# Guilucand/PanDelos

Hardware: AMD Instinct MI355X
Metric: scored gene-pairs/sec (whole node) (higher is better)
Workload: dtype u32 accumulate + f32 finalize

## Files before the change

### pandelos_amd/csrc/pdl_api.hip

```cpp
#include "pdl_common.h"

#include <algorithm>
#include <cstdlib>
#include <cstring>
#include <limits>

static thread_local std::string g_create_error = "";


static void check_genes(const char *who, const uint8_t *residues, const uint64_t *offsets, uint32_t n) {
    if (!offsets) PDL_FAIL(PDL_ERR_ARGUMENT, "%s: NULL pointer", who);
    if (n == 0) PDL_FAIL(PDL_ERR_ARGUMENT, "%s: no gene", who);
    for (uint32_t i = 0; i < n; i++)
        if (offsets[i + 1] < offsets[i]) PDL_FAIL(PDL_ERR_ARGUMENT, "%s: offsets decrease at gene %u", who, i);
    if (!residues && offsets[n] > offsets[0]) PDL_FAIL(PDL_ERR_ARGUMENT, "%s: NULL residues", who);
}

static void check_batch(const pdl_ctx *c, const char *who, const void *out, const uint8_t *residues, const uint64_t *offsets, const uint32_t *gene_begin,
                        uint32_t n, uint32_t n_queries) {
    if (n_queries == 0) PDL_FAIL(PDL_ERR_ARGUMENT, "%s: no query", who);
    if (n == 0) PDL_FAIL(PDL_ERR_ARGUMENT, "%s: no query gene", who);
    if (!out || !offsets || !gene_begin) PDL_FAIL(PDL_ERR_ARGUMENT, "%s: NULL pointer", who);
    if (gene_begin[0] != 0) PDL_FAIL(PDL_ERR_ARGUMENT, "%s: gene_begin[0] = %u, not 0", who, gene_begin[0]);
    for (uint32_t q = 0; q < n_queries; q++)
// ... 744 lines not shown
}

int pdl_set_option(pdl_ctx *c, const char *name, int64_t value) {
    if (!c || !name) return PDL_ERR_ARGUMENT;
    std::lock_guard<std::mutex> lk(c->mu);
    return guarded(c, [&]() -> int {
    const std::string n(name);
    if (n == "join_tier1") {
        if (!(value == -1 || value == 0 || (value >= 9 && value <= 11) || value == 20 || value == 21)) PDL_FAIL(PDL_ERR_ARGUMENT, "join_tier1: -1, 0, 9, 10, 11, 20 or 21");
        c->opt_tier1 = (int) value;
    } else if (n == "join_tier0") c->opt_tier0 = value < 0 ? -1 : (value != 0);
    else if (n == "sift_threshold") {
        if (value != 0 && value != 1) PDL_FAIL(PDL_ERR_ARGUMENT, "sift_threshold: 0 or 1");
        c->opt_sift_threshold = (int) value;
    }
    else if (n == "join_tiny_tier2") c->opt_tiny_tier2 = value != 0;
    else if (n == "join_grid_pct") c->opt_grid_pct = (int) value;
    else if (n == "stage_timers") c->opt_stage_timers = value != 0;
    else if (n == "host_mirror") c->opt_host_mirror = value != 0;
    else if (n == "staging_cap") c->opt_staging_cap = value > 0 ? (uint64_t) value : 0;
    else if (n == "aside_test_reload") c->opt_aside_test_reload = value != 0;
    else if (n == "onepass_scan") c->opt_onepass_scan = value != 0;
    else if (n == "lean_radix") c->opt_lean_radix = value != 0;
    else if (n == "low_memory") c->opt_low_memory = value != 0;
    else if (n == "query_batch_bytes") {
        if (value <= 0) PDL_FAIL(PDL_ERR_ARGUMENT, "query_batch_bytes: a positive byte count");
        c->opt_query_batch_bytes = (uint64_t) value;
        return PDL_OK;
    }
    else if (n == "query_rekey") {
        if (value != 0 && value != 1) PDL_FAIL(PDL_ERR_ARGUMENT, "query_rekey: 0 or 1");
        c->opt_query_rekey = value != 0;
        return PDL_OK;
    }
    else if (n == "alphabet_rekey") {
        if (value != 0 && value != 1) PDL_FAIL(PDL_ERR_ARGUMENT, "alphabet_rekey: 0 or 1");
        c->opt_alphabet_rekey = value != 0;
        return PDL_OK;
    }
    else throw pdl_error{PDL_ERR_ARGUMENT, "unknown option " + n};
    pdl_stale(c, Stale::scores);
    return PDL_OK;
    });
}

int pdl_dist_preprocess_begin(pdl_ctx *c, const uint8_t *d_residues, const uint64_t *d_offsets, const uint32_t *d_genome_of,
// ... 274 lines not shown
```

### pandelos_amd/csrc/pdl_common.h

```cpp
#pragma once

#include <atomic>
#include <chrono>

#include <hip/hip_runtime.h>

#include <algorithm>
#include <cstdint>
#include <cstdio>
#include <mutex>
#include <cstdlib>
#include <new>
#include <string>
#include <utility>
#include <vector>

#include "../../include/pandelos_amd.h"

#define PDL_WAVE 64

#ifdef __HIPCC__
__device__ __forceinline__ void pdl_sync() {
#ifndef PDL_PLAIN_SYNCTHREADS
    asm volatile("s_waitcnt lgkmcnt(0)" ::: "memory");
#endif
    __syncthreads();
}
#endif

enum : size_t {
    PDL_CTL_RECORDS = 0,
    PDL_CTL_FREE_1 = 1,
    PDL_CTL_RANGES = 2,
    PDL_CTL_BAD_OFFSETS = 3,
    PDL_CTL_KSEQ_SUM = 4,
    PDL_CTL_KMERS = 5,
    PDL_CTL_EMITTED = 6,
    PDL_CTL_KSEQ_MAX = 7,
    PDL_CTL_KSEQ_NMIN = 8,
    PDL_CTL_MIRRORED = 9,
    PDL_CTL_COUNTERS = 10,
    PDL_CTL_SHARED = 10,
// ... 276 lines not shown

    DevBuf kseq_len;
    DevBuf gene_len;
    DevBuf kmer_off;
    DevBuf cost;
    std::vector<uint64_t> h_genome_cost;

    DevBuf keys_a, keys_b, vals_a, vals_b, sort_tmp;
    bool key64 = false;
    DevBuf recpos;
    DevBuf post;
    DevBuf ranges;
    const uint2 *ranges8 = nullptr;
    DevBuf head_bits;
    bool costs_ready = true;
    DevBuf seq_off;
    bool upper_only = false;
    DevBuf scan_tmp;
    DevBuf lb_tile, lb_chunk, lb_ctr;
    uint32_t lb_epoch = 0;
    bool opt_low_memory = false;
    bool reshard_pending = false;
    bool opt_onepass_scan = false;
    bool opt_lean_radix = true;
    DevBuf scratch;
    DevBuf scalars;

    std::vector<uint32_t> h_genome_of;
    std::vector<uint32_t> h_genome_row_off;
    std::vector<uint32_t> h_genome_rows;
    std::vector<uint32_t> shard;
    bool shard_set = false;
    std::vector<uint32_t> dict_shard;
    DevBuf seq_in_shard;
    DevBuf own_iv;
    std::vector<uint2> h_own_iv;
    std::vector<uint8_t> h_seq_in_shard;

    bool scored = false;
    uint32_t n_task_rows = 0;
    std::vector<int32_t> h_local_genome;
    std::vector<uint32_t> h_task_row_off;
    std::vector<uint64_t> h_cell_off;
    DevBuf task_blob;
    uint32_t *task_pin = nullptr; size_t task_pin_words = 0;
    hipStream_t copy_stream = nullptr; hipEvent_t ev_tasks = nullptr, ev_entry = nullptr;
// ... 391 lines not shown
```

### pandelos_amd/csrc/pdl_dict.hip

```cpp
#include "pdl_common.h"
#include "pdl_scan.h"
#include "pdl_sort.h"
#include "pdl_append.h"
#include "pdl_remove.h"
#include "pdl_rekey.h"
#include "pdl_groups.h"

#include <algorithm>
#include <cstring>


__global__ __launch_bounds__(256) void k_zero_u64(uint64_t *p, size_t n) {
    for (size_t i = (size_t) blockIdx.x * 256 + threadIdx.x; i < n; i += (size_t) gridDim.x * 256) p[i] = 0;
}
constexpr int HIST_THREADS = 256;
__global__ __launch_bounds__(HIST_THREADS) void k_hist(const uint8_t *__restrict__ res, uint64_t n, unsigned long long *__restrict__ hist) {
    __shared__ uint32_t s_seen[256];
    s_seen[threadIdx.x] = 0;
    pdl_sync();
    const uint64_t n16 = n / 16;
    const uint4 *res16 = reinterpret_cast<const uint4 *>(res);
    const uint64_t stride = (uint64_t) gridDim.x * HIST_THREADS;
    auto mark = [&](const uint4 &v) {
        const uint32_t w[4] = {v.x, v.y, v.z, v.w};
// ... 649 lines not shown
    c->tm.sort_seq_ms = ev_ms(c, EV_SORT2); c->tm.ranges_ms = ev_ms(c, EV_RANGES);
    return ev_ms(c, total_event);
}

static void stage_ranges_and_costs(pdl_ctx *c, uint64_t bound, int mode, bool only_complexity) {
    uint64_t *d_scal = c->scalars.as<uint64_t>();
    GroupPlan gp = group_tiles_plan(c, pdl_postings(c), bound, d_scal + PDL_CTL_RECORDS);
    gp.a.cost = c->cost.as<unsigned long long>();
    gp.a.counters = reinterpret_cast<unsigned long long *>(d_scal + PDL_CTL_COUNTERS);
    hipLaunchKernelGGL(k_fold_last_record, dim3(1), dim3(1024), 0, c->stream, gp.a.post, c->post_ext ? (uint32_t *) nullptr : c->recpos.as<uint32_t>(), gp.a.d_n);
    if (only_complexity) { c->ranges8 = nullptr; launch_group_costs<false, true>(c, gp.a, gp.grid); }
    else build_ranges(c, gp.a, gp.grid, mode);
    c->costs_ready = c->ranges8 == nullptr;
    launch_genome_cost(c, PDL_CTL_KSEQ_SUM, PDL_CTL_KSEQ_MAX);
    PinRead rd(c);
    const uint64_t *pt = closing_read(c, rd, PDL_CTL_GCOST + (size_t) c->G);
    c->h_genome_cost.assign(pt + PDL_CTL_GCOST, pt + PDL_CTL_GCOST + c->G);
    c->U = pt[PDL_CTL_RECORDS]; c->Ushared = pt[PDL_CTL_SHARED]; c->Urepeat = pt[PDL_CTL_REPEATS]; c->NG = pt[PDL_CTL_GROUPS];
    c->P = c->costs_ready ? 0 : pt[PDL_CTL_OWN_COST];
    if (c->costs_ready) for (uint64_t v : c->h_genome_cost) c->P += v;
}

void pdl_run_reshard(pdl_ctx *c) {
    hipStream_t st = c->stream;
    if (c->dist || c->post_ext) PDL_FAIL(PDL_ERR_STATE, "genome shard: a multi-GPU context deals the genomes itself");
    if (c->dict_shard.empty() || c->upper_only) PDL_FAIL(PDL_ERR_STATE, "genome shard: the dictionary was built for all genomes; set the first shard before pdl_preprocess");
    const uint32_t n = (uint32_t) c->U;
    ev_begin(c, EV_PRE_TOTAL);
    hipLaunchKernelGGL(k_restore_heads, dim3((n + 255) / 256), dim3(256), 0, st, c->post.as<uint2>(), c->head_bits.as<unsigned long long>(), n);
    clear_ctl(c, PDL_CTL_RANGES, PDL_CTL_RANGES);
    clear_ctl(c, PDL_CTL_COUNTERS, PDL_CTL_LAST);
    clear_genome_words(c);
    clear_gene_costs(c);
    const uint64_t sum_kseq = c->sum_kseq, max_kseq = c->max_kseq, min_kseq = c->min_kseq;
    clear_kseq_stats(c);
    c->dict_shard = c->shard;
    c->tasks_ready = false;
    ev_begin(c, EV_DICT); ev_end(c, EV_DICT);
    stage_ranges_and_costs(c, c->U, 0, false);
    c->sum_kseq = sum_kseq; c->max_kseq = max_kseq; c->min_kseq = min_kseq;
    ev_end(c, EV_PRE_TOTAL);
    c->tm.reshard_ms = close_range_timings(c, EV_PRE_TOTAL);
}

void pdl_ensure_costs(pdl_ctx *c) {
    if (c->costs_ready) return;
    hipStream_t st = c->stream;
    uint64_t *d_scal = c->scalars.as<uint64_t>();
    clear_gene_costs(c);
    clear_genome_words(c, false);
    const uint32_t n = (uint32_t) c->U;
    hipLaunchKernelGGL(k_gene_costs_lazy, dim3((n + 255) / 256), dim3(256), 0, st, pdl_postings(c), c->head_bits.as<unsigned long long>(), n,
// ... 688 lines not shown
```

### pandelos_amd/csrc/pdl_groups.h

```cpp
#pragma once
#include "pdl_common.h"
#include "pdl_scan.h"
#include "pdl_sort.h"

constexpr uint32_t HEAD_BIT = 0x80000000u;
constexpr uint32_t GT_NONE = 0xffffffffu;
constexpr uint32_t COST_LDS_GENOMES = 4096;
constexpr int GW_ROUNDS = 16, GW_TILE = GW_ROUNDS * PDL_WAVE, GW_THREADS = 256, GW_WAVES = GW_THREADS / PDL_WAVE;
constexpr uint32_t GW_MAX_IV = 2048;

__device__ __forceinline__ uint32_t find_head_back(const uint2 *post, uint32_t pos, uint32_t lane) {
    for (;;) {
        const uint32_t base = pos + 1 >= PDL_WAVE ? pos + 1 - PDL_WAVE : 0;
        const uint32_t idx = base + lane;
        const bool f = idx <= pos && ((post[idx <= pos ? idx : pos].y >> 31) || idx == 0);
        const unsigned long long m = __ballot(f);
        if (m) return base + 63u - (uint32_t) __clzll((long long) m);
        pos = base - 1;
    }
}
__device__ __forceinline__ uint32_t find_head_fwd(const uint2 *post, uint32_t pos, uint32_t n, uint32_t lane) {
    for (uint32_t base = pos; base < n; base += PDL_WAVE) {
        const uint32_t idx = base + lane;
        const bool f = idx < n && (post[idx < n ? idx : n - 1].y >> 31);
// ... 195 lines not shown
            if (hm) { after = (uint32_t) __shfl((int) v, __ffsll((long long) hm) - 1, PDL_WAVE); break; }
        }
    }
    before = (uint32_t) __builtin_amdgcn_readfirstlane((int) before);
    after = (uint32_t) __builtin_amdgcn_readfirstlane((int) after);
}

__device__ __forceinline__ void gt_next_heads(const unsigned long long (&m)[GW_ROUNDS], uint32_t t0, uint32_t after, uint32_t (&nextr)[GW_ROUNDS]) {
    uint32_t nx = after;
#pragma unroll
    for (int j = GW_ROUNDS - 1; j >= 0; j--) {
        nextr[j] = nx;
        if (m[j]) nx = t0 + j * PDL_WAVE + (uint32_t) __ffsll((long long) m[j]) - 1u;
    }
}
__device__ __forceinline__ void gt_round_extent(unsigned long long mj, uint32_t r0, uint32_t lane, uint32_t nextr_j, uint32_t &pr, uint32_t &gs, uint32_t &ge) {
    const unsigned long long le_mask = (2ull << lane) - 1ull;
    const unsigned long long at_or_below = mj & le_mask, above = mj & ~le_mask;
    gs = at_or_below ? r0 + 63u - (uint32_t) __clzll((long long) at_or_below) : pr;
    ge = above ? r0 + (uint32_t) __ffsll((long long) above) - 1u : nextr_j;
    if (mj) pr = r0 + 63u - (uint32_t) __clzll((long long) mj);
}

__device__ __forceinline__ uint32_t gt_take_head(const GroupTileArgs &a, uint32_t tile, int j, uint32_t u, bool live, uint32_t y, unsigned long long mj, uint32_t lane) {
    const uint32_t cnt = y & ~HEAD_BIT;
    if (live && (y >> 31)) a.post[u].y = cnt;
    if (a.head_bits && lane == 0) a.head_bits[(size_t) tile * GW_ROUNDS + j] = mj;
    return cnt;
}

__device__ __forceinline__ unsigned long long gt_pack_range(uint32_t start, uint32_t len, uint32_t cnt, uint32_t pos_base) {
    return (unsigned long long) (start + pos_base) | ((unsigned long long) (len | (min(cnt, 1023u) << 22)) << 32);
}

template <bool GENOMES, bool RECORD_COSTS>
__global__ __launch_bounds__(GW_THREADS) void k_group_costs(GroupTileArgs a) {
    __shared__ uint32_t s_red[2];
    extern __shared__ unsigned long long s_dyn[];
    unsigned long long *s_full = s_dyn, *s_upper = s_dyn + a.n_genomes;
    const uint32_t tid = threadIdx.x, lane = tid & (PDL_WAVE - 1);
    const uint32_t gw = blockIdx.x * GW_WAVES + tid / PDL_WAVE;
    const uint32_t n = (uint32_t) scan_count(a.n_bound, a.d_n);
    const uint32_t tiles = (n + GW_TILE - 1) / GW_TILE;
    const bool lds_table = GENOMES && a.n_genomes <= COST_LDS_GENOMES;
    if constexpr (GENOMES) { if (lds_table) { for (uint32_t i = tid; i < 2 * a.n_genomes; i += GW_THREADS) s_dyn[i] = 0; } }
    if (tid < 2) s_red[tid] = 0;
    pdl_sync();
    uint32_t n_rec = 0, n_grp = 0;
    for (uint32_t tile = gw; tile < tiles; tile += gridDim.x * GW_WAVES) {
        const uint32_t t0 = tile * GW_TILE, t1 = min(t0 + (uint32_t) GW_TILE, n);
        uint2 po[GW_ROUNDS];
// ... 41 lines not shown
}

__global__ __launch_bounds__(256) void k_gene_costs_lazy(const uint2 *__restrict__ post, const unsigned long long *__restrict__ head_bits,
                                                         uint32_t n, unsigned long long *__restrict__ cost) {
    const uint32_t u = blockIdx.x * 256 + threadIdx.x;
    if (u >= n) return;
    const uint32_t w = u >> 6, b = u & 63u, words = (n + 63) >> 6;
    uint32_t gs, ge;
    {
        unsigned long long m = head_bits[w] & ((2ull << b) - 1ull);
        uint32_t ww = w;
        while (!m && ww > 0) m = head_bits[--ww];
        gs = m ? ww * 64u + 63u - (uint32_t) __clzll((long long) m) : 0u;
    }
    {
        unsigned long long m = b == 63 ? 0ull : head_bits[w] & ~((2ull << b) - 1ull);
        uint32_t ww = w;
        while (!m && ww + 1 < words) m = head_bits[++ww];
        ge = m ? ww * 64u + (uint32_t) __ffsll((long long) m) - 1u : n;
        if (ge > n) ge = n;
    }
    if (ge - gs >= 2) atomicAdd(&cost[post[u].x], (unsigned long long) (ge - gs));
}
__global__ __launch_bounds__(256) void k_restore_heads(uint2 *__restrict__ post, const unsigned long long *__restrict__ head_bits, uint32_t n) {
    const uint32_t u = blockIdx.x * 256 + threadIdx.x;
    if (u >= n) return;
    if ((head_bits[u >> 6] >> (u & 63u)) & 1ull) post[u].y |= HEAD_BIT;
}

template <int MODE>
__global__ __launch_bounds__(GW_THREADS) void k_range_count(GroupTileArgs a) {
    extern __shared__ unsigned long long s_dyn[];
    __shared__ uint32_t s_red[2];
    uint2 *s_iv = reinterpret_cast<uint2 *>(s_dyn);
    const uint32_t n_iv = (MODE == 0 || MODE == 2) ? a.n_own_iv : 0u;
    if constexpr (MODE == 0 || MODE == 2) { for (uint32_t i = threadIdx.x; i < n_iv; i += GW_THREADS) s_iv[i] = a.own_iv[i]; }
    if (threadIdx.x < 2) s_red[threadIdx.x] = 0;
    pdl_sync();
    const uint32_t tid = threadIdx.x, lane = tid & (PDL_WAVE - 1);
    const uint32_t gw = blockIdx.x * GW_WAVES + tid / PDL_WAVE;
    const uint32_t n = (uint32_t) scan_count(a.n_bound, a.d_n);
    const uint32_t tiles = (n + GW_TILE - 1) / GW_TILE;
    uint32_t n_rec = 0, n_grp = 0, n_rep = 0;
    for (uint32_t tile = gw; tile < tiles; tile += gridDim.x * GW_WAVES)
        gt_count_tile<MODE, false>(a, tile, n, lane, s_iv, n_iv, nullptr, n_rec, n_grp, n_rep);
    gt_flush_counts<true>(a, s_red, n_rec, n_grp, n_rep);
}

static_assert(GW_WAVES * GW_TILE == (int) PDL_RADIX_TILE && GW_THREADS == (int) PDL_RADIX_BINS, "a workgroup's four tiles are one tile of the radix pass");
__global__ __launch_bounds__(GW_THREADS) void k_range_count_hist(GroupTileArgs a, uint32_t n_tiles4, uint32_t *__restrict__ counts) {
    __shared__ uint32_t s_h[PDL_RADIX_BINS];
// ... 34 lines not shown
        gt_load_tile(a.post, t0, n, lane, po);
        uint32_t hb, ha;
        gt_load_borders(a, tile, tiles, lane, hb, ha);
        const uint32_t ins = gt_shard_mask<MODE>(a, s_iv, n_iv, po);
        unsigned long long m[GW_ROUNDS];
        gt_head_masks(po, t0, n, lane, m);
        uint32_t before, after;
        gt_tile_borders(a, tile, tiles, t0, n, m[0], lane, hb, ha, before, after);
        uint32_t nextr[GW_ROUNDS];
        gt_next_heads(m, t0, after, nextr);
        uint32_t pr = before, cnt_tile = 0;
        const uint32_t tile_prefix = a.chunk_sums[tile / PDL_WAVE] + a.tile_sums[tile];
#pragma unroll
        for (int j = 0; j < GW_ROUNDS; j++) {
            const uint32_t u = t0 + j * PDL_WAVE + lane;
            uint32_t gs, ge;
            gt_round_extent(m[j], t0 + j * PDL_WAVE, lane, nextr[j], pr, gs, ge);
            const bool live = u < n;
            const bool shared = live && ge - gs >= 2;
            const bool mine = MODE == 1 || ((ins >> j) & 1u);
            bool r = shared && mine;
            if constexpr (MODE == 1 || MODE == 2) r = r && u + 1 < ge;
            const unsigned long long rb = __ballot(r);
            const uint32_t cnt = gt_take_head(a, tile, j, u, live, po[j].y, m[j], lane);
            if (live) {
                if (shared && mine) own_lookups += ge - gs;
                if (r) {
                    const uint32_t at = tile_prefix + cnt_tile + (uint32_t) __popcll(rb & lt_mask);
                    const uint32_t start = MODE == 0 ? gs : u + 1;
                    a.key2[at] = po[j].x;
                    if (a.pay8) a.pay8[at] = gt_pack_range(start, ge - start, cnt, a.pos_base);
                    else a.tuples[at] = make_uint4(start, ge - start, cnt, ge - gs);
                } else if (MODE == 1 || MODE == 2) {
                    if (!a.pay8 && ge - gs >= 2 && u + 1 == ge && mine) atomicAdd(&a.cost[po[j].x], (unsigned long long) (ge - gs));
                }
            }
            cnt_tile += (uint32_t) __popcll(rb);
        }
    }
#pragma unroll
    for (int d = PDL_WAVE / 2; d > 0; d >>= 1) own_lookups += __shfl_xor(own_lookups, d, PDL_WAVE);
    if (lane == 0 && own_lookups) atomicAdd(&s_own, own_lookups);
    pdl_sync();
    if (tid == 0 && s_own) atomicAdd(&a.counters[2], s_own);
}

__global__ __launch_bounds__(GW_THREADS) void k_range_scatter(GroupTileArgs a, uint32_t n_tiles4, const uint32_t *__restrict__ offs,
// ... 20 lines not shown
    unsigned long long val[GW_ROUNDS];
    uint16_t rank[GW_ROUNDS];
    uint32_t rbits = 0;
    unsigned long long own_lookups = 0;
    gt_load_tile(a.post, t0, n, lane, po);
    if (active) {
        uint32_t hb, ha;
        gt_load_borders(a, tile, tiles, lane, hb, ha);
        unsigned long long m[GW_ROUNDS];
        gt_head_masks(po, t0, n, lane, m);
        uint32_t before, after;
        gt_tile_borders(a, tile, tiles, t0, n, m[0], lane, hb, ha, before, after);
        uint32_t nextr[GW_ROUNDS];
        gt_next_heads(m, t0, after, nextr);
        uint32_t pr = before;
#pragma unroll
        for (int j = 0; j < GW_ROUNDS; j++) {
            const uint32_t u = t0 + j * PDL_WAVE + lane;
            uint32_t gs, ge;
            gt_round_extent(m[j], t0 + j * PDL_WAVE, lane, nextr[j], pr, gs, ge);
            const bool live = u < n;
            const bool shared = live && ge - gs >= 2;
            const bool r = shared && u + 1 < ge;
            const uint32_t cnt = gt_take_head(a, tile, j, u, live, po[j].y, m[j], lane);
            if (shared) own_lookups += ge - gs;
            val[j] = gt_pack_range(u + 1, ge - u - 1, cnt, 0u);
            rbits |= (uint32_t) r << j;
        }
    }
    uint32_t key[GW_ROUNDS];
#pragma unroll
    for (int j = 0; j < GW_ROUNDS; j++) key[j] = po[j].x;
    const auto valid = [&](int j) { return (rbits >> j) & 1u; };
    radix_rank_rounds<8>(s.cnt[wave], key, 0u, valid, rank);
    pdl_sync();
    uint32_t grand_total;
    const uint32_t tile_total = radix_tile_layout(s, goff, dtot, grand_total);
    if (digit_total && blockIdx.x == 0 && tid == 0) *d_total = grand_total;
    pdl_sync();
    radix_tile_place(s, wave, key, val, 0u, valid, rank);
#pragma unroll
    for (int d = PDL_WAVE / 2; d > 0; d >>= 1) own_lookups += __shfl_xor(own_lookups, d, PDL_WAVE);
    if (lane == 0 && own_lookups) atomicAdd(&s_own, own_lookups);
    pdl_sync();
    radix_tile_write(s, 0u, tile_total, keys_out, vals_out);
    if (tid == 0 && s_own) atomicAdd(&a.counters[2], s_own);
}
// ... 51 lines not shown
```

### pandelos_amd/csrc/pdl_join.hip

```cpp
#include "pdl_common.h"
#include "pdl_scan.h"

#include <algorithm>
#include <cstdlib>
#include <cstring>

constexpr int HBM_THREADS = 512;
constexpr uint32_t EMPTY_KEY = 0xffffffffu;
constexpr uint64_t FIELD_MASK = (1ull << 21) - 1;
constexpr uint32_t CELL_CHUNK = 16384;

struct JoinArgs {
    const uint2 *post;
    const uint4 *ranges;
    const uint2 *ranges8;
    const uint32_t *seq_off;
    const uint32_t *kseq_len;
    const uint32_t *genome_of;
    const uint4 *gene_info;
    const uint32_t *task_rows;
    const uint32_t *task_lg;
    const uint32_t *work;
    const uint4 *desc;
    uint32_t n_work;
// ... 245 lines not shown
            const uint32_t i = tid * RPT + j;
            s_cum[i] = i < nb ? ex : (i == nb ? total : 0xffffffffu);
            if (len[j]) {
                uint32_t w_lo = 0;
                if constexpr (NW <= 4) {
#pragma unroll
                    for (uint32_t w = 0; w < NW; w++) w_lo += (uint32_t) (w * seg < ex);
                } else {
                    w_lo = seg ? (ex + seg - 1) / seg : 0;
                }
                for (uint32_t w = w_lo; w < NW && w * seg < ex + len[j]; w++) s_wstart[w] = make_uint2(i, ex);
            }
            ex += len[j];
        }
        if (tid == 0) s_cum[RB] = nb == RB ? total : 0xffffffffu;
        pdl_sync();
        return total;
    };
    const bool packed = a.ranges8 != nullptr;
    auto unpack = [&](uint2 &gm, uint32_t &gsv, uint32_t r, bool live) {
        if (packed) {
            gsv = gm.x + (gm.y & 0x3fffffu);
            gm.y >>= 22;
            if (__builtin_expect(gm.y == 1023u && live, 0)) gm.y = a.post[gm.x - 1].y;
        } else gsv = s_gsv[r];
    };
    auto walk = [&](uint32_t total, auto &&fn4) {
        constexpr uint32_t NW = T / PDL_WAVE;
        const uint32_t lane = tid & (PDL_WAVE - 1), wave = tid / PDL_WAVE;
        const uint32_t chunks = (total + PDL_WAVE - 1) / PDL_WAVE;
        const uint32_t cpw = (chunks + NW - 1) / NW;
        uint32_t ch = wave * cpw;
        const uint32_t ch_end = min(chunks, ch + cpw);
        if (ch >= ch_end) return;
        const uint2 ws = s_wstart[wave];
        uint32_t rs = __builtin_amdgcn_readfirstlane(ws.x);
        for (; ch < ch_end; ch += NCH) {
            if (*(volatile uint32_t *) &s_overflow) break;
            uint2 gm[NCH], po[NCH];
            uint32_t adr[NCH], gsv[NCH];
            bool live[NCH];
            const uint32_t nu = min(NCH, ch_end - ch);
            const uint32_t f_lo = ch * PDL_WAVE, f_hi = f_lo + nu * PDL_WAVE;
            const uint32_t vw = s_cum[rs + 1 + lane];
            if (__builtin_amdgcn_readlane(vw, PDL_WAVE - 1) >= f_hi) {
#pragma unroll
                for (uint32_t u = 0; u < NCH; u++) {
// ... 25 lines not shown
                    const uint32_t f0 = (ch + u) * PDL_WAVE, f = f0 + lane;
                    const uint32_t v = s_cum[rs + 1 + lane];
                    const bool inside = v < f0 + PDL_WAVE;
                    const int recv = __builtin_amdgcn_ds_permute((int) ((inside ? v - f0 : 0u) << 2), inside ? 1 : 0);
                    const unsigned long long m = __ballot(recv != 0);
                    const uint32_t w = (uint32_t) __popcll(__ballot(inside));
                    const uint32_t r = rs + __builtin_amdgcn_mbcnt_hi((uint32_t) (m >> 32), __builtin_amdgcn_mbcnt_lo((uint32_t) m, 0u)) + (uint32_t) (recv != 0);
                    const uint32_t off = f - s_cum[r];
                    live[u] = f < total;
                    gm[u] = s_gm[r];
                    adr[u] = gm[u].x + off;
                    unpack(gm[u], gsv[u], r, live[u]);
#ifdef PDL_JOIN_CHECK
                    if (live[u] && !(s_cum[r] <= f && f < s_cum[r + 1] && off == f - s_cum[r])) atomicAdd(a.error_count, 1000u);
#endif
                    const uint32_t nextb = w < PDL_WAVE ? __builtin_amdgcn_readlane(v, w) : s_cum[rs + 1 + PDL_WAVE];
                    rs += w + (uint32_t) (nextb == f0 + PDL_WAVE);
                }
            }
            }
            PH_WAIT(); PH_MARK(5);
#pragma unroll
            for (uint32_t u = 0; u < NCH; u++) po[u] = a.post[live[u] ? adr[u] : 0u];
            PH_WAIT(); PH_MARK(6);
#ifdef PDL_JOIN_CHECK
            if (*(volatile uint32_t *) &s_rowseq != my_seq) atomicAdd(a.error_count, 1000000u);
#endif
            fn4(po, gm, gsv, live);
#ifdef PDL_JOIN_CHECK
            if (*(volatile uint32_t *) &s_rowseq != my_seq) atomicAdd(a.error_count, 1000000u);
#endif
        }
    };

    for (;;) {
        pdl_sync();
        const uint32_t wi = s_next;
        const uint4 d = s_desc;
#ifdef PDL_JOIN_CHECK
        my_seq++;
        if (tid == 0) s_rowseq = my_seq;
#endif
        pdl_sync();
        PH_MARK(0);
        if (wi >= n_work) break;
        uint32_t next_reg = 0;
// ... 245 lines not shown
    if (tid == 0) { s_ntouched = 0; s_nemit = 0; s_work = 0xffffffffu; s_batch_end = 0; }
    const float threshold = 1.0f / (2.0f * (float) a.k);
    const uint32_t n_work = a.n_work_ptr ? *a.n_work_ptr : a.n_work;
    pdl_sync();
    for (;;) {
        if (tid == 0) {
            uint32_t nx = s_work + 1;
            if (nx >= s_batch_end) { nx = atomicAdd(a.work_cursor, a.work_batch); s_batch_end = nx + a.work_batch; }
            s_work = nx;
        }
        pdl_sync();
        const uint32_t wi = s_work;
        if (wi >= n_work) break;
        const uint32_t p = a.work[wi];
        const uint32_t r = a.task_rows[p];
        const uint32_t e0 = a.seq_off[r], e1 = a.seq_off[r + 1];
        const uint32_t wave = tid / PDL_WAVE, lane = tid % PDL_WAVE, nwaves = JOIN_THREADS / PDL_WAVE;
        for (uint32_t e = e0 + wave; e < e1; e += nwaves) {
            uint4 rg;
            uint32_t group_key;
            if (a.ranges8) {
                const uint2 r8 = a.ranges8[e];
                uint32_t own = r8.y >> 22;
                if (own == 1023u) own = a.post[r8.x - 1].y;
                rg = make_uint4(r8.x, r8.y & 0x3fffffu, own, 0u);
                group_key = rg.x + rg.y;
            } else {
                rg = a.ranges[e];
                group_key = rg.x + rg.y - rg.w;
            }
            const uint32_t finv = 0xffffffffu - group_key;
            for (uint32_t q = lane; q < rg.y; q += PDL_WAVE) {
                const uint2 po = a.post[rg.x + q];
                const uint32_t c = po.x;
                if (ld_agent(&t_first[c]) < finv) {
                    const uint32_t old = atomicMax(&t_first[c], finv);
                    if (old == 0) {
                        const uint32_t idx = atomicAdd(&s_ntouched, 1u);
                        if (idx < a.N) t_touched[idx] = c; else atomicAdd(a.error_count, 1u);
                    }
                }
                if constexpr (WIDE) {
                    atomicAdd(&t_w[c], min(po.y, rg.z));
                    atomicAdd(&t_w[a.N + c], rg.z);
                    atomicAdd(&t_w[2 * (size_t) a.N + c], po.y);
                } else {
                    const unsigned long long add = (unsigned long long) min(po.y, rg.z) | ((unsigned long long) rg.z << 21) | ((unsigned long long) po.y << 42);
                    atomicAdd(&t_acc[c], add);
                }
            }
        }
        __threadfence();
        asm volatile("s_waitcnt vmcnt(0)" ::: "memory");
        pdl_sync();
        const uint32_t ntouched = min(s_ntouched, a.N);
        const uint32_t my_kcnt = a.kseq_len[r];
// ... 423 lines not shown
    const uint32_t p = blockIdx.x * 256 + threadIdx.x;
    if (p < n_genes) {
        const uint32_t g = genome_of[p];
        gene_info[p] = make_uint4(kseq_len[p], g, taskpos_of[p], local_genome[g]);
    }
    if (p >= n_rows) return;
    const uint32_t r = task_rows[p];
    const uint32_t e0 = seq_off[r];
    desc[p] = make_uint4(p, r, e0, seq_off[r + 1] - e0);
}

struct RowCntFlag {
    const uint32_t *row_cnt; const uint32_t *mirror_cnt;
    __device__ uint32_t operator()(uint64_t p) const { return row_cnt[p] + (mirror_cnt ? mirror_cnt[p] : 0u); }
};
struct MirrorCntFlag {
    const uint32_t *mirror_cnt;
    __device__ uint32_t operator()(uint64_t p) const { return mirror_cnt[p]; }
};
struct FinOffApply {
    uint32_t *fin_off;
    __device__ void operator()(uint64_t p, uint32_t, uint32_t prefix) const { fin_off[p] = prefix; }
};
__global__ void k_gather_u32(const uint32_t *src, const uint32_t *idx, uint32_t n, uint32_t *dst, const uint32_t *ctr, const uint32_t *z64) {
    uint32_t i = blockIdx.x * blockDim.x + threadIdx.x;
    if (i < n) dst[i] = src[idx[i]];
    else if (i < n + PDL_JT_CTR_WORDS) dst[i] = ctr[i - n];
    else if (i < n + PDL_JT_EMITTED + 2) dst[i] = z64[i - n - PDL_JT_EMITTED];
    else if (i == n + PDL_JT_RELOADS) dst[i] = ctr[PDL_JC_RELOADS];
    else if (i == n + PDL_JT_ROWS_T1) dst[i] = ctr[PDL_JC_ROWS_T1];
}

struct ZeroRanges { uint4 *p[4]; unsigned long long n16[4]; };
__global__ __launch_bounds__(256) void k_zero_ranges(ZeroRanges z) {
    const unsigned long long stride = (unsigned long long) gridDim.x * 256;
#pragma unroll
    for (int r = 0; r < 4; r++)
        for (unsigned long long i = (unsigned long long) blockIdx.x * 256 + threadIdx.x; i < z.n16[r]; i += stride) z.p[r][i] = make_uint4(0, 0, 0, 0);
}

void pdl_prepare_tasks(pdl_ctx *c) {
    hipStream_t st = c->stream;
    const uint32_t N = c->N, G = c->G;
    if (!c->shard_set) { c->shard.resize(G); for (uint32_t g = 0; g < G; g++) c->shard[g] = g; }
    const uint32_t S = (uint32_t) c->shard.size();
    c->h_local_genome.assign(G, -1);
// ... 281 lines not shown
}

struct JoinCounters {
    uint32_t rows_tier2, rows_tier3, reloads;
    unsigned long long cells;
};
static JoinCounters join_counters(const uint32_t *w, bool inbox_filed = false) {
    if (w[PDL_JC_ERRORS] && inbox_filed)
        PDL_FAIL(PDL_ERR_ARGUMENT, "pdl_dist_score_finish: %u received cells name a gene beyond the set or a column that is not a row of this rank; begin the pass again (pdl_dist_score_begin)", w[PDL_JC_ERRORS]);
    if (w[PDL_JC_ERRORS]) PDL_FAIL(PDL_ERR_DEVICE, "join: %u internal consistency violations", w[PDL_JC_ERRORS]);
    JoinCounters j{w[PDL_JC_ROWS_T2], w[PDL_JC_ROWS_T3], w[PDL_JC_RELOADS], 0};
    memcpy(&j.cells, w + PDL_JC_CELLS, sizeof(j.cells));
    return j;
}

static unsigned long long score_order(pdl_ctx *c, const ScorePlan &pl, const pdl_dist_cell *d_inbox, uint32_t n_inbox, int ev_total) {
    hipStream_t st = c->stream;
    const uint32_t n_rows = c->n_task_rows;
    const uint32_t S = (uint32_t) c->shard.size();
    uint64_t *d_scal = c->scalars.as<uint64_t>();
    uint32_t *ctr32 = c->join_ctr.as<uint32_t>();
    ev_begin(c, EV_ORDER);
    const uint32_t *d_mcnt = pl.mirror ? c->mirror_cnt.as<uint32_t>() : nullptr;
    scan_and_apply(c, n_rows, RowCntFlag{c->row_cnt.as<uint32_t>(), d_mcnt}, FinOffApply{c->fin_off.as<uint32_t>()}, d_scal + PDL_CTL_EMITTED,
                   reinterpret_cast<uint64_t *>(c->fin_off.as<uint32_t>() + n_rows));
    OrderArgs o{};
    if (pl.mirror) {
        uint32_t *m_off = c->mirror_cnt.as<uint32_t>() + n_rows, *m_cur = m_off + n_rows;
        scan_and_apply(c, n_rows, MirrorCntFlag{d_mcnt}, FinOffApply{m_off}, d_scal + PDL_CTL_MIRRORED);
        MirrorArgs ma{};
        set_staged_cells(ma, staged_cells(c));
        ma.taskpos_of = c->taskpos_of.as<uint32_t>(); ma.mirror_off = m_off; ma.mirror_cur = m_cur; ma.n_rows = n_rows;
        ma.mcell = c->mirror_ref.as<MCell>();
        hipLaunchKernelGGL(k_mirror_cells, dim3((n_rows + 3) / 4), dim3(256), 0, st, ma);
        if (n_inbox) hipLaunchKernelGGL(k_mirror_cells_inbox, dim3((n_inbox + 255) / 256), dim3(256), 0, st, ma, d_inbox, n_inbox, c->N);
        o.mirror_cnt = d_mcnt; o.mirror_off = m_off; o.mcell = c->mirror_ref.as<MCell>();
    }
    set_staged_cells(o, staged_cells(c)); o.fin_off = c->fin_off.as<uint32_t>();
    o.c_score = c->c_score.as<float>(); o.c_perc = c->c_perc.as<float>(); o.c_tr = c->c_tr.as<float>();
    o.c_row = c->c_row.as<int32_t>(); o.c_col = c->c_col.as<int32_t>();
    o.n_rows = n_rows; o.canonical = (c->flags & PDL_FLAG_CANONICAL_ORDER) ? 1u : 0u; o.pack_ok = c->N < (1u << 22) ? 1u : 0u;
    o.wide_rows = ctr32 + PDL_JC_WIDE_ROWS;
    launch_order(c, o);
    PDL_HIP(hipGetLastError());
    ev_end(c, EV_ORDER);

    uint32_t *d_idx = c->task_off.as<uint32_t>();
    uint32_t *d_out = d_idx + (S + 1);
    hipLaunchKernelGGL(k_gather_u32, dim3((S + 1 + PDL_JT_WORDS + 255) / 256), dim3(256), 0, st, c->fin_off.as<uint32_t>(), d_idx, S + 1, d_out,
                       ctr32, reinterpret_cast<const uint32_t *>(d_scal + PDL_CTL_EMITTED));
    c->h_fin.resize(S + 1);
    JoinCounters jc;
// ... 188 lines not shown
```

### pandelos_amd/csrc/pdl_join_part.h

```cpp
#pragma once

constexpr uint32_t PT_T = 256;
constexpr uint32_t PT_T2 = 512, PT_WGS2 = 3;
constexpr uint32_t PT_RB = 960;
constexpr uint32_t PT_ROWS = 4;
#ifndef PT_WG_PER_CU
#define PT_WG_PER_CU 5
#endif
constexpr uint32_t PT_NCH = 4, PT_ITERS = PT_WG_PER_CU >= 5 ? 4 : 6;
constexpr uint32_t PT_KPT = PT_NCH * PT_ITERS;
constexpr uint32_t PT_HEAVY_CAP = 64;
constexpr uint32_t PT_BM_BITS = PT_WG_PER_CU >= 5 ? 10 : 11, PT_BM_WORDS = 1u << PT_BM_BITS;
constexpr uint32_t PT_CNT_WORDS = 2 * PT_BM_WORDS;
constexpr uint32_t PT_CNT_SHIFT = 22 - (PT_BM_BITS + 2);
constexpr uint32_t PT_T_MAX = 255;
constexpr uint32_t PT_BM_SHIFT = 22 - PT_BM_BITS;
#ifndef PT_SIFT_T_MIN
#define PT_SIFT_T_MIN 4
#endif
constexpr uint32_t PT_HT_BITS = 10, PT_HT = 1u << PT_HT_BITS;
constexpr uint32_t PT_BATCH = 8;
constexpr uint32_t PT_HASH_MUL = 0x9E3779B1u & 0x3fffffu;
constexpr uint32_t pt_inverse(uint32_t m) { uint32_t x = m; for (int i = 0; i < 5; i++) x *= 2u - m * x; return x; }
constexpr uint32_t PT_HASH_INV = pt_inverse(PT_HASH_MUL);
// ... 286 lines not shown
                                const uint32_t w = (uint32_t) __popcll(__ballot(inside));
                                const uint32_t r = rs + __builtin_amdgcn_mbcnt_hi((uint32_t) (m >> 32), __builtin_amdgcn_mbcnt_lo((uint32_t) m, 0u)) + (uint32_t) (recv != 0);
                                live[u] = f < total;
                                const uint32_t rl = live[u] ? r : 0u;
                                const uint2 gmu = s_gm[rl];
                                const uint32_t cum_r = s_cum[rl];
                                key[it * PT_NCH + u] = rl;
                                adr[u] = gmu.x + (f - cum_r);
                                ownhv |= (uint32_t) ((gmu.y >> 22) >= 2u) << u;
                                const uint32_t nextb = w < PDL_WAVE ? (uint32_t) __builtin_amdgcn_readlane((int) v, w) : s_cum[rs + 1 + PDL_WAVE];
                                rs += w + (uint32_t) (nextb == f0 + PDL_WAVE);
                            }
                        }
                    }
#pragma unroll
                    for (uint32_t u = 0; u < PT_NCH; u++) po[u] = a.post[live[u] ? adr[u] : 0u];
                    if constexpr (CNT) {
#pragma unroll
                        for (uint32_t u = 0; u < PT_NCH; u++) {
                            const uint32_t h = pt_mul_u24(po[u].x, PT_HASH_MUL) & 0x3fffffu;
                            key[it * PT_NCH + u] |= h << 10;
                            const uint32_t ci = h >> PT_CNT_SHIFT;
                            uint32_t add = 1u;
                            if (live[u] && (po[u].y >= 2u || ((ownhv >> u) & 1u))) {
                                const uint32_t i = atomicAdd(&s_nheavy, 1u);
                                add = i < PT_HEAVY_CAP ? sift_t : 0u;
                                if (i < PT_HEAVY_CAP) s_heavy[i] = make_uint2(key[it * PT_NCH + u], po[u].y);
                            }
                            if (live[u]) atomicAdd(&s_cnt[ci >> 1], add << ((ci & 1u) << 4));
                        }
                    } else {
                    uint32_t seen[PT_NCH], bit[PT_NCH], wd[PT_NCH];
#pragma unroll
                    for (uint32_t u = 0; u < PT_NCH; u++) {
                        const uint32_t h = pt_mul_u24(po[u].x, PT_HASH_MUL) & 0x3fffffu;
                        key[it * PT_NCH + u] |= h << 10;
                        wd[u] = h >> PT_BM_SHIFT; bit[u] = 1u << ((h >> (PT_BM_SHIFT - 5)) & 31u);
                        seen[u] = live[u] ? atomicOr(&s_bm1[wd[u]], bit[u]) : 0u;
                        if (live[u] && (po[u].y >= 2u || ((ownhv >> u) & 1u))) {
                            seen[u] = bit[u];
                            const uint32_t i = atomicAdd(&s_nheavy, 1u);
                            if (i < PT_HEAVY_CAP) s_heavy[i] = make_uint2(key[it * PT_NCH + u], po[u].y);
                        }
                    }
#pragma unroll
                    for (uint32_t u = 0; u < PT_NCH; u++) if (seen[u] & bit[u]) atomicOr(&s_bm2[wd[u]], bit[u]);
                    }
                }
                ch += PT_NCH;
            }
        }
        pdl_sync();
        PT_MARK(3);
        uint32_t *wlist = (CNT ? s_cum : s_bm1) + wave * PT_WLIST;
        uint32_t nsv = 0;
        const uint32_t n_heavy = uni(s_nheavy);
        if (n_heavy > PT_HEAVY_CAP) s_overflow = 1;
        auto drain = [&](bool all) {
            asm volatile("s_waitcnt lgkmcnt(0)" ::: "memory");
            const uint32_t i_lo = all ? 0u : nsv % (2 * PDL_WAVE);
            for (uint32_t i0 = i_lo; i0 < nsv; i0 += 2 * PDL_WAVE) {
                const uint32_t ia = i0 + lane, ib = ia + PDL_WAVE;
                const uint32_t ka = wlist[ia < nsv ? ia : 0u], kb = wlist[ib < nsv ? ib : 0u];
                if (ia < nsv) add_one(ka);
                if (ib < nsv) add_one(kb);
// ... 50 lines not shown
            unsigned long long nx = s_chunk_next;
            if (nx + ntouched > s_chunk_end) {
                nx = atomicAdd(a.cell_cursor, (unsigned long long) CELL_CHUNK);
                s_chunk_end = nx + CELL_CHUNK;
            }
            s_base = nx;
        }
        pdl_sync();
        const unsigned long long base = s_base;
        const bool fits = base + ntouched <= a.st_cap;
        const uint32_t c0 = uni(s_tslot[0]), c1 = uni(s_tslot[1]), c2 = uni(s_tslot[2]);
        const uint32_t sb1 = c0, sb2 = c0 + c1, sb3 = c0 + c1 + c2;
        for (uint32_t t = tid; t < ntouched; t += PT_T) {
            const uint32_t ts = s_touched[t];
            const uint32_t w = s_tkey[ts] - 1u, light = s_tn[ts];
            s_tkey[ts] = 0u; s_tn[ts] = 0u;
            const uint32_t hk = w >> 10, minr = w & 1023u, sl = ts >> sub_bits;
            uint32_t s_min = 0, s_own = 0, s_cc = 0;
            for (uint32_t e = 0; e < n_heavy; e++) {
                const uint2 hv = s_heavy[e];
                if ((hv.x >> 10) == hk && slot_of(hv.x & 1023u) == sl) {
                    const uint2 g = s_gm[hv.x & 1023u];
                    uint32_t own = g.y >> 22;
                    if (own == 1023u) own = a.post[g.x - 1].y;
                    s_min += min(hv.y, own) - 1u; s_own += own - 1u; s_cc += hv.y - 1u;
                }
            }
            const uint32_t inter = light + s_min, pcn = light + s_own, tcn = light + s_cc;
            const PartRow row = s_row[sl];
            const uint32_t c = (hk * PT_HASH_INV) & 0x3fffffu;
            if (c >= a.N) { atomicAdd(a.error_count, 1u); continue; }
            if (c == row.r) continue;
            if (pcn < row.pc_min && tcn < tc_min) continue;
            const uint4 ci4 = a.gene_info[c];
            float perc, tr;
            const float score = finalize_counts((int) inter, (int) pcn, (int) tcn, row.kcnt, ci4.x, threshold, perc, tr);
            if (score > 0.0f) {
                const uint32_t i = atomicAdd(&s_nemit[sl], 1u);
                if (fits) {
                    const unsigned long long o = base + (sl == 0 ? 0u : sl == 1 ? sb1 : sl == 2 ? sb2 : sb3) + i;
                    const uint2 g = s_gm[minr];
                    a.st_score[o] = score; a.st_perc[o] = perc; a.st_tr[o] = tr;
                    a.st_col[o] = c; a.st_first[o] = track_first ? g.x + (g.y & 0x3fffffu) : 0xffffffffu;
                    const uint32_t gc = ci4.y;
                    atomicMax(reinterpret_cast<uint32_t *>(a.MS + (size_t) row.p * a.G + gc), __float_as_uint(score));
                    atomicMax(reinterpret_cast<uint32_t *>(a.CM + (size_t) row.lg * a.N + c), __float_as_uint(score));
                    if (a.mirror) {
// ... 36 lines not shown
```

Before: 1533 billion.

## Fuse order offset scans into one kernel and keep head bits in postings

Result: no change. 1558 billion, median of 6 (+1.6%).

```diff
diff --git a/pandelos_amd/csrc/pdl_api.hip b/pandelos_amd/csrc/pdl_api.hip
--- a/pandelos_amd/csrc/pdl_api.hip
+++ b/pandelos_amd/csrc/pdl_api.hip
@@ -790,6 +790,14 @@
     else if (n == "aside_test_reload") c->opt_aside_test_reload = value != 0;
     else if (n == "onepass_scan") c->opt_onepass_scan = value != 0;
     else if (n == "lean_radix") c->opt_lean_radix = value != 0;
+    else if (n == "order_offsets") {
+        if (value < 0 || value > 2) PDL_FAIL(PDL_ERR_ARGUMENT, "order_offsets: 0 (two scans), 1 (one workgroup) or 2 (several)");
+        c->opt_order_offsets = (int) value;
+    }
+    else if (n == "order_offsets_rows") {
+        if (value < 0) PDL_FAIL(PDL_ERR_ARGUMENT, "order_offsets_rows: a row count");
+        c->opt_order_offsets_rows = (uint32_t) std::min<int64_t>(value, 0xffffffffll);
+    }
     else if (n == "low_memory") c->opt_low_memory = value != 0;
     else if (n == "query_batch_bytes") {
         if (value <= 0) PDL_FAIL(PDL_ERR_ARGUMENT, "query_batch_bytes: a positive byte count");
diff --git a/pandelos_amd/csrc/pdl_common.h b/pandelos_amd/csrc/pdl_common.h
--- a/pandelos_amd/csrc/pdl_common.h
+++ b/pandelos_amd/csrc/pdl_common.h
@@ -18,6 +18,8 @@
 #include "../../include/pandelos_amd.h"
 
 #define PDL_WAVE 64
+
+constexpr uint32_t PDL_COUNT_MASK = 0x7fffffffu;
 
 #ifdef __HIPCC__
 __device__ __forceinline__ void pdl_sync() {
@@ -340,6 +342,8 @@
     bool opt_low_memory = false;
     bool reshard_pending = false;
     bool opt_onepass_scan = false;
+    int opt_order_offsets = 2;
+    uint32_t opt_order_offsets_rows = 1u << 17;
     bool opt_lean_radix = true;
     DevBuf scratch;
     DevBuf scalars;
diff --git a/pandelos_amd/csrc/pdl_dict.hip b/pandelos_amd/csrc/pdl_dict.hip
--- a/pandelos_amd/csrc/pdl_dict.hip
+++ b/pandelos_amd/csrc/pdl_dict.hip
@@ -695,12 +695,9 @@
 }
 
 void pdl_run_reshard(pdl_ctx *c) {
-    hipStream_t st = c->stream;
     if (c->dist || c->post_ext) PDL_FAIL(PDL_ERR_STATE, "genome shard: a multi-GPU context deals the genomes itself");
     if (c->dict_shard.empty() || c->upper_only) PDL_FAIL(PDL_ERR_STATE, "genome shard: the dictionary was built for all genomes; set the first shard before pdl_preprocess");
-    const uint32_t n = (uint32_t) c->U;
     ev_begin(c, EV_PRE_TOTAL);
-    hipLaunchKernelGGL(k_restore_heads, dim3((n + 255) / 256), dim3(256), 0, st, c->post.as<uint2>(), c->head_bits.as<unsigned long long>(), n);
     clear_ctl(c, PDL_CTL_RANGES, PDL_CTL_RANGES);
     clear_ctl(c, PDL_CTL_COUNTERS, PDL_CTL_LAST);
     clear_genome_words(c);
diff --git a/pandelos_amd/csrc/pdl_groups.h b/pandelos_amd/csrc/pdl_groups.h
--- a/pandelos_amd/csrc/pdl_groups.h
+++ b/pandelos_amd/csrc/pdl_groups.h
@@ -241,11 +241,9 @@
     if (mj) pr = r0 + 63u - (uint32_t) __clzll((long long) mj);
 }
 
-__device__ __forceinline__ uint32_t gt_take_head(const GroupTileArgs &a, uint32_t tile, int j, uint32_t u, bool live, uint32_t y, unsigned long long mj, uint32_t lane) {
-    const uint32_t cnt = y & ~HEAD_BIT;
-    if (live && (y >> 31)) a.post[u].y = cnt;
+__device__ __forceinline__ uint32_t gt_take_head(const GroupTileArgs &a, uint32_t tile, int j, uint32_t y, unsigned long long mj, uint32_t lane) {
     if (a.head_bits && lane == 0) a.head_bits[(size_t) tile * GW_ROUNDS + j] = mj;
-    return cnt;
+    return y & PDL_COUNT_MASK;
 }
 
 __device__ __forceinline__ unsigned long long gt_pack_range(uint32_t start, uint32_t len, uint32_t cnt, uint32_t pos_base) {
@@ -333,11 +331,6 @@
     }
     if (ge - gs >= 2) atomicAdd(&cost[post[u].x], (unsigned long long) (ge - gs));
 }
-__global__ __launch_bounds__(256) void k_restore_heads(uint2 *__restrict__ post, const unsigned long long *__restrict__ head_bits, uint32_t n) {
-    const uint32_t u = blockIdx.x * 256 + threadIdx.x;
-    if (u >= n) return;
-    if ((head_bits[u >> 6] >> (u & 63u)) & 1ull) post[u].y |= HEAD_BIT;
-}
 
 template <int MODE>
 __global__ __launch_bounds__(GW_THREADS) void k_range_count(GroupTileArgs a) {
@@ -418,7 +411,7 @@
             bool r = shared && mine;
             if constexpr (MODE == 1 || MODE == 2) r = r && u + 1 < ge;
             const unsigned long long rb = __ballot(r);
-            const uint32_t cnt = gt_take_head(a, tile, j, u, live, po[j].y, m[j], lane);
+            const uint32_t cnt = gt_take_head(a, tile, j, po[j].y, m[j], lane);
             if (live) {
                 if (shared && mine) own_lookups += ge - gs;
                 if (r) {
@@ -485,7 +478,7 @@
             const bool live = u < n;
             const bool shared = live && ge - gs >= 2;
             const bool r = shared && u + 1 < ge;
-            const uint32_t cnt = gt_take_head(a, tile, j, u, live, po[j].y, m[j], lane);
+            const uint32_t cnt = gt_take_head(a, tile, j, po[j].y, m[j], lane);
             if (shared) own_lookups += ge - gs;
             val[j] = gt_pack_range(u + 1, ge - u - 1, cnt, 0u);
             rbits |= (uint32_t) r << j;
diff --git a/pandelos_amd/csrc/pdl_join.hip b/pandelos_amd/csrc/pdl_join.hip
--- a/pandelos_amd/csrc/pdl_join.hip
+++ b/pandelos_amd/csrc/pdl_join.hip
@@ -291,7 +291,7 @@
         if (packed) {
             gsv = gm.x + (gm.y & 0x3fffffu);
             gm.y >>= 22;
-            if (__builtin_expect(gm.y == 1023u && live, 0)) gm.y = a.post[gm.x - 1].y;
+            if (__builtin_expect(gm.y == 1023u && live, 0)) gm.y = a.post[gm.x - 1].y & PDL_COUNT_MASK;
         } else gsv = s_gsv[r];
     };
     auto walk = [&](uint32_t total, auto &&fn4) {
@@ -363,6 +363,8 @@
             PH_WAIT(); PH_MARK(5);
 #pragma unroll
             for (uint32_t u = 0; u < NCH; u++) po[u] = a.post[live[u] ? adr[u] : 0u];
+#pragma unroll
+            for (uint32_t u = 0; u < NCH; u++) po[u].y &= PDL_COUNT_MASK;
             PH_WAIT(); PH_MARK(6);
 #ifdef PDL_JOIN_CHECK
             if (*(volatile uint32_t *) &s_rowseq != my_seq) atomicAdd(a.error_count, 1000000u);
@@ -654,7 +656,7 @@
             if (a.ranges8) {
                 const uint2 r8 = a.ranges8[e];
                 uint32_t own = r8.y >> 22;
-                if (own == 1023u) own = a.post[r8.x - 1].y;
+                if (own == 1023u) own = a.post[r8.x - 1].y & PDL_COUNT_MASK;
                 rg = make_uint4(r8.x, r8.y & 0x3fffffu, own, 0u);
                 group_key = rg.x + rg.y;
             } else {
@@ -663,7 +665,8 @@
             }
             const uint32_t finv = 0xffffffffu - group_key;
             for (uint32_t q = lane; q < rg.y; q += PDL_WAVE) {
-                const uint2 po = a.post[rg.x + q];
+                uint2 po = a.post[rg.x + q];
+                po.y &= PDL_COUNT_MASK;
                 const uint32_t c = po.x;
                 if (ld_agent(&t_first[c]) < finv) {
                     const uint32_t old = atomicMax(&t_first[c], finv);
@@ -1133,6 +1136,97 @@
     uint32_t *fin_off;
     __device__ void operator()(uint64_t p, uint32_t, uint32_t prefix) const { fin_off[p] = prefix; }
 };
+constexpr uint32_t OO_THREADS = 1024, OO_ITEMS = 4, OO_TILE = OO_THREADS * OO_ITEMS;
+constexpr uint32_t OO_MAX_ROWS = 1u << 17;
+__device__ __forceinline__ unsigned long long oo_pack(uint32_t cells, uint32_t mirrored) { return ((unsigned long long) cells << 32) + mirrored; }
+__device__ __forceinline__ unsigned long long oo_block_scan(unsigned long long v, unsigned long long extra, unsigned long long *s_wave ,
+                                                            unsigned long long *s_extra , unsigned long long &total, unsigned long long &extra_total) {
+    constexpr uint32_t NW = OO_THREADS / PDL_WAVE;
+    const uint32_t lane = threadIdx.x & (PDL_WAVE - 1), wave = threadIdx.x / PDL_WAVE;
+    unsigned long long inc = v;
+#pragma unroll
+    for (int d = 1; d < PDL_WAVE; d <<= 1) {
+        const unsigned long long o = __shfl_up(inc, d, PDL_WAVE);
+        if (lane >= (uint32_t) d) inc += o;
+    }
+#pragma unroll
+    for (int d = PDL_WAVE / 2; d > 0; d >>= 1) extra += __shfl_xor(extra, d, PDL_WAVE);
+    if (lane == PDL_WAVE - 1) { s_wave[wave] = inc; s_extra[wave] = extra; }
+    pdl_sync();
+    if (threadIdx.x < PDL_WAVE) {
+        const unsigned long long w = lane < NW ? s_wave[lane] : 0ull;
+        unsigned long long winc = w, e = lane < NW ? s_extra[lane] : 0ull;
+#pragma unroll
+        for (int d = 1; d < (int) NW; d <<= 1) {
+            const unsigned long long o = __shfl_up(winc, d, PDL_WAVE);
+            if (lane >= (uint32_t) d) winc += o;
+        }
+#pragma unroll
+        for (int d = (int) NW / 2; d > 0; d >>= 1) e += __shfl_xor(e, d, PDL_WAVE);
+        if (lane < NW) s_wave[lane] = winc - w;
+        if (lane == NW - 1) s_wave[16] = winc;
+        if (lane == 0) s_extra[0] = e;
+    }
+    pdl_sync();
+    const unsigned long long res = inc - v + s_wave[wave];
+    total = s_wave[16]; extra_total = s_extra[0];
+    pdl_sync();
+    return res;
+}
+__global__ __launch_bounds__(OO_THREADS) void k_order_offsets(const uint32_t *__restrict__ row_cnt, const uint32_t *__restrict__ mirror_cnt, uint32_t n_rows,
+                                                              uint32_t span, uint32_t *__restrict__ fin_off, uint32_t *__restrict__ m_off,
+                                                              uint64_t *d_emitted, uint64_t *d_mirrored) {
+    __shared__ unsigned long long s_wave[17], s_extra[16];
+    const uint32_t tid = threadIdx.x;
+    const uint32_t r0 = min(blockIdx.x * span, n_rows), r1 = min(r0 + span, n_rows);
+    unsigned long long carry = 0;
+    for (uint32_t base = r0; base < r1; base += OO_TILE) {
+        const uint32_t i0 = base + tid * OO_ITEMS;
+        const bool whole = i0 + OO_ITEMS <= r1;
+        uint32_t f[OO_ITEMS], m[OO_ITEMS];
+        if (whole) {
+            const uint4 rc = *reinterpret_cast<const uint4 *>(row_cnt + i0), mc = *reinterpret_cast<const uint4 *>(mirror_cnt + i0);
+            m[0] = mc.x; m[1] = mc.y; m[2] = mc.z; m[3] = mc.w;
+            f[0] = rc.x + mc.x; f[1] = rc.y + mc.y; f[2] = rc.z + mc.z; f[3] = rc.w + mc.w;
+        } else {
+#pragma unroll
+            for (uint32_t j = 0; j < OO_ITEMS; j++) {
+                const bool live = i0 + j < r1;
+                m[j] = live ? mirror_cnt[i0 + j] : 0u;
+                f[j] = live ? row_cnt[i0 + j] + m[j] : 0u;
+            }
+        }
+        uint32_t pc = 0, pm = 0;
+        if (base == r0) {
+            const uint32_t n4 = r0 / 4;
+            const uint4 *rc4 = reinterpret_cast<const uint4 *>(row_cnt), *mc4 = reinterpret_cast<const uint4 *>(mirror_cnt);
+#pragma unroll 8
+            for (uint32_t i = tid; i < n4; i += OO_THREADS) {
+                const uint4 a = rc4[i], b = mc4[i];
+                pc += a.x + a.y + a.z + a.w; pm += b.x + b.y + b.z + b.w;
+            }
+        }
+        unsigned long long sum = 0, total, front;
+#pragma unroll
+        for (uint32_t j = 0; j < OO_ITEMS; j++) sum += oo_pack(f[j], m[j]);
+        unsigned long long ex = oo_block_scan(sum, oo_pack(pc + pm, pm), s_wave, s_extra, total, front);
+        carry += front;
+        ex += carry;
+#pragma unroll
+        for (uint32_t j = 0; j < OO_ITEMS; j++) {
+            if (i0 + j < r1) { fin_off[i0 + j] = (uint32_t) (ex >> 32); m_off[i0 + j] = (uint32_t) ex; }
+            ex += oo_pack(f[j], m[j]);
+        }
+        carry += total;
+    }
+    if (blockIdx.x == gridDim.x - 1 && tid == 0) {
+        const uint32_t cells = (uint32_t) (carry >> 32);
+        *d_emitted = cells;
+        fin_off[n_rows] = cells; fin_off[n_rows + 1] = 0u;
+        *d_mirrored = (uint32_t) carry;
+    }
+}
+
 __global__ void k_gather_u32(const uint32_t *src, const uint32_t *idx, uint32_t n, uint32_t *dst, const uint32_t *ctr, const uint32_t *z64) {
     uint32_t i = blockIdx.x * blockDim.x + threadIdx.x;
     if (i < n) dst[i] = src[idx[i]];
@@ -1460,12 +1554,19 @@
     uint32_t *ctr32 = c->join_ctr.as<uint32_t>();
     ev_begin(c, EV_ORDER);
     const uint32_t *d_mcnt = pl.mirror ? c->mirror_cnt.as<uint32_t>() : nullptr;
-    scan_and_apply(c, n_rows, RowCntFlag{c->row_cnt.as<uint32_t>(), d_mcnt}, FinOffApply{c->fin_off.as<uint32_t>()}, d_scal + PDL_CTL_EMITTED,
-                   reinterpret_cast<uint64_t *>(c->fin_off.as<uint32_t>() + n_rows));
+    const bool one_launch = pl.mirror && c->opt_order_offsets != 0 && n_rows > 0 && n_rows <= std::min(c->opt_order_offsets_rows, OO_MAX_ROWS);
+    if (one_launch) {
+        const uint32_t span = c->opt_order_offsets == 1 ? (n_rows + OO_TILE - 1) / OO_TILE * OO_TILE : OO_TILE;
+        hipLaunchKernelGGL(k_order_offsets, dim3((n_rows + span - 1) / span), dim3(OO_THREADS), 0, st, c->row_cnt.as<uint32_t>(), d_mcnt, n_rows, span,
+                           c->fin_off.as<uint32_t>(), c->mirror_cnt.as<uint32_t>() + n_rows, d_scal + PDL_CTL_EMITTED, d_scal + PDL_CTL_MIRRORED);
+    } else {
+        scan_and_apply(c, n_rows, RowCntFlag{c->row_cnt.as<uint32_t>(), d_mcnt}, FinOffApply{c->fin_off.as<uint32_t>()}, d_scal + PDL_CTL_EMITTED,
+                       reinterpret_cast<uint64_t *>(c->fin_off.as<uint32_t>() + n_rows));
+    }
     OrderArgs o{};
     if (pl.mirror) {
         uint32_t *m_off = c->mirror_cnt.as<uint32_t>() + n_rows, *m_cur = m_off + n_rows;
-        scan_and_apply(c, n_rows, MirrorCntFlag{d_mcnt}, FinOffApply{m_off}, d_scal + PDL_CTL_MIRRORED);
+        if (!one_launch) scan_and_apply(c, n_rows, MirrorCntFlag{d_mcnt}, FinOffApply{m_off}, d_scal + PDL_CTL_MIRRORED);
         MirrorArgs ma{};
         set_staged_cells(ma, staged_cells(c));
         ma.taskpos_of = c->taskpos_of.as<uint32_t>(); ma.mirror_off = m_off; ma.mirror_cur = m_cur; ma.n_rows = n_rows;
diff --git a/pandelos_amd/csrc/pdl_join_part.h b/pandelos_amd/csrc/pdl_join_part.h
--- a/pandelos_amd/csrc/pdl_join_part.h
+++ b/pandelos_amd/csrc/pdl_join_part.h
@@ -332,10 +332,10 @@
                             key[it * PT_NCH + u] |= h << 10;
                             const uint32_t ci = h >> PT_CNT_SHIFT;
                             uint32_t add = 1u;
-                            if (live[u] && (po[u].y >= 2u || ((ownhv >> u) & 1u))) {
+                            if (live[u] && ((po[u].y & PDL_COUNT_MASK) >= 2u || ((ownhv >> u) & 1u))) {
                                 const uint32_t i = atomicAdd(&s_nheavy, 1u);
                                 add = i < PT_HEAVY_CAP ? sift_t : 0u;
-                                if (i < PT_HEAVY_CAP) s_heavy[i] = make_uint2(key[it * PT_NCH + u], po[u].y);
+                                if (i < PT_HEAVY_CAP) s_heavy[i] = make_uint2(key[it * PT_NCH + u], po[u].y & PDL_COUNT_MASK);
                             }
                             if (live[u]) atomicAdd(&s_cnt[ci >> 1], add << ((ci & 1u) << 4));
                         }
@@ -347,10 +347,10 @@
                         key[it * PT_NCH + u] |= h << 10;
                         wd[u] = h >> PT_BM_SHIFT; bit[u] = 1u << ((h >> (PT_BM_SHIFT - 5)) & 31u);
                         seen[u] = live[u] ? atomicOr(&s_bm1[wd[u]], bit[u]) : 0u;
-                        if (live[u] && (po[u].y >= 2u || ((ownhv >> u) & 1u))) {
+                        if (live[u] && ((po[u].y & PDL_COUNT_MASK) >= 2u || ((ownhv >> u) & 1u))) {
                             seen[u] = bit[u];
                             const uint32_t i = atomicAdd(&s_nheavy, 1u);
-                            if (i < PT_HEAVY_CAP) s_heavy[i] = make_uint2(key[it * PT_NCH + u], po[u].y);
+                            if (i < PT_HEAVY_CAP) s_heavy[i] = make_uint2(key[it * PT_NCH + u], po[u].y & PDL_COUNT_MASK);
                         }
                     }
 #pragma unroll
@@ -447,7 +447,7 @@
                 if ((hv.x >> 10) == hk && slot_of(hv.x & 1023u) == sl) {
                     const uint2 g = s_gm[hv.x & 1023u];
                     uint32_t own = g.y >> 22;
-                    if (own == 1023u) own = a.post[g.x - 1].y;
+                    if (own == 1023u) own = a.post[g.x - 1].y & PDL_COUNT_MASK;
                     s_min += min(hv.y, own) - 1u; s_own += own - 1u; s_cc += hv.y - 1u;
                 }
             }
```
